# dsilvestro/npBNN

Hardware: AMD Instinct MI355X
Metric: MCMC iterations/sec (full fwd+lik per proposal) (higher is better)
Workload: dtype f16x3-split/f32

## Files before the change

npbnn_amd/csrc/npbnn_eval.hip.h:

```cpp
#pragma once
#include "npbnn_common.hip.h"
#include "npbnn_chain.hip.h"

namespace npbnn {

typedef void (*eval_fn_t)(const EvalParams*, int, int);
constexpr int kLikCat = 0, kLikGauss = 1, kLikGen = 2;
__host__ __device__ inline int lik_class(int lik_kind) {
    return lik_needs_row_scratch(lik_kind) ? kLikGen : (lik_kind == NPBNN_LIK_GAUSS ? kLikGauss : kLikCat);
}

template <int LK>
struct TileAcc {
    double ll;
};
template <>
struct TileAcc<kLikGauss> {
    double s1[4], s2[4];
};
constexpr int kFastGaussTargets = 2;

__device__ __forceinline__ int uni(int v) { return __builtin_amdgcn_readfirstlane(v); }
__device__ __forceinline__ float uni(float v) { return __uint_as_float(__builtin_amdgcn_readfirstlane(__float_as_uint(v))); }
__device__ __forceinline__ long long uni(long long v) {
    const unsigned lo = __builtin_amdgcn_readfirstlane((unsigned)(unsigned long long)v);
    const unsigned hi = __builtin_amdgcn_readfirstlane((unsigned)((unsigned long long)v >> 32));
    return (long long)(((unsigned long long)hi << 32) | lo);
}
template <typename T>
__device__ __forceinline__ T* uni(T* ptr) { return reinterpret_cast<T*>(uni((long long)reinterpret_cast<unsigned long long>(ptr))); }

#ifndef NPBNN_LAUNDER_TID
#define NPBNN_LAUNDER_TID (FAST && !SPEC && (BLK || (LK == kLikGauss && MT0 >= 2) || MT0 >= 3))
#endif
#ifndef NPBNN_LAUNDER_TAIL
#define NPBNN_LAUNDER_TAIL (FAST && !SPEC && (BLK || (LK == kLikGauss && MT0 >= 2) || MT0 >= 3))
#endif
#ifndef NPBNN_FAST3_WAVES
#define NPBNN_FAST3_WAVES 12
#endif
constexpr int kFastMaxMT0 = 4;
constexpr int kFastLayers = 3;
struct HotParams {
    const int* labels;
    const float* targets;
    const float* inst_w;
    unsigned* confusion;
    float* y_out;
    long long n_rows;
    int use_classw, predict_mode, weight_sets;
    int aux_off_w, aux_off_t;
    int n_layers, C, MTL, lik_kind, k_targets, act_kind, out_kind, final_act, classw_off, pad_masked;
    int slope_off;
    int l1_f16;
    int frag_off[kFastLayers - 1], bias_off[kFastLayers - 1], in_live[kFastLayers - 1];
    float act_prm[kFastLayers - 1];
};

template <int KIND, int HT, int D>
__device__ __forceinline__ void act_tiles_all(f32x4 (&h)[D][HT], int live, float prm) {
#pragma unroll
    for (int mt = 0; mt < HT; ++mt)
        if (mt < live)
#pragma unroll
            for (int i = 0; i < 4; ++i)
#pragma unroll
                for (int j = 0; j < D; ++j) h[j][mt][i] = act_apply(h[j][mt][i], KIND, prm);
}
template <int HT, int D>
__device__ __forceinline__ void act_live_all(f32x4 (&h)[D][HT], int live, int kind, float prm) {
    switch (kind) {
        case NPBNN_ACT_RELU: act_tiles_all<NPBNN_ACT_RELU>(h, live, prm); break;
        case NPBNN_ACT_LEAKY: act_tiles_all<NPBNN_ACT_LEAKY>(h, live, prm); break;
        case NPBNN_ACT_SWISH: act_tiles_all<NPBNN_ACT_SWISH>(h, live, prm); break;
        default: act_tiles_all<NPBNN_ACT_TANH>(h, live, prm); break;
    }
}

template <int MT0, int MTI, int LK, int D, int DA, int J0, int NLC = 0, int ACTC = -1, bool PLAIN = false, bool F16IMG = false, int GT = 0>
__device__ __forceinline__ void tile_tail(const NetMeta& net, const HotParams& hp, const float* imgs0, int image_floats,
                                          const f32x4 (&acc0_all)[DA][MT0], int lane, int n, int kq, const char* a_slot, float* row_scratch,
                                          long long row, bool row_ok, TileAcc<LK> (&A_all)[DA]) {
    static_assert(J0 + D <= DA, "candidate range");
    constexpr bool primary = J0 == 0;
    const float* const imgs = imgs0 + (size_t)J0 * image_floats;
    auto A = [&](int j) -> TileAcc<LK>& { return A_all[J0 + j]; };
    constexpr int HT = MT0 > MTI ? MT0 : MTI;
    static_assert(NLC == 0 || (MTI == 1 && NLC >= 2 && NLC <= kFastLayers), "shape-specialised tails: 2..kFastLayers layers, narrow later layers");
    static_assert(!PLAIN || (NLC > 0 && LK != kLikGen), "the plain form needs a fixed shape");
    const int n_layers = NLC ? NLC : hp.n_layers;
    const int C = hp.C;
    const int MTL = NLC ? 1 : hp.MTL;
    const int lik_kind = (PLAIN && LK == kLikCat) ? NPBNN_LIK_CATEGORICAL : hp.lik_kind;
    const int k_targets = hp.k_targets;
    const bool need_softmax = LK == kLikCat && (PLAIN || (lik_kind == NPBNN_LIK_CATEGORICAL) || (hp.predict_mode == 2 && hp.out_kind == NPBNN_OUT_SOFTMAX));
    f32x4 h[D][HT];
#pragma unroll
    for (int j = 0; j < D; ++j)
#pragma unroll
        for (int mt = 0; mt < HT; ++mt) h[j][mt] = mt < MT0 ? acc0_all[J0 + j][mt < MT0 ? mt : 0] : f32x4{0.f, 0.f, 0.f, 0.f};
    auto layer = [&](int lkt, int lmt, int frag_off, int bias_off, float prm, int hidden, int live_s) {
        if constexpr (ACTC >= 0) {
            act_tiles_all<ACTC>(h, lkt, prm);
        } else if (hp.slope_off >= 0) {
#pragma unroll
            for (int j = 0; j < D; ++j) act_live(h[j], lkt, hp.act_kind, imgs[(size_t)j * image_floats + hp.slope_off + hidden]);
        } else {
            act_live_all(h, lkt, hp.act_kind, prm);
        }
        const float* frag = imgs + frag_off + lane * 4;
        const float* bias = imgs + bias_off + 4 * kq;
        f32x4 acc[D][MTI];
#pragma unroll
        for (int mt = 0; mt < MTI; ++mt) {
#pragma unroll
            for (int j = 0; j < D; ++j) acc[j][mt] = f32x4{0.f, 0.f, 0.f, 0.f};
            if (mt < lmt) {
#pragma unroll
                for (int j = 0; j < D; ++j) acc[j][mt] = *reinterpret_cast<const f32x4*>(bias + (size_t)j * image_floats + 16 * mt);
#pragma unroll
                for (int ct = 0; ct < HT; ++ct) {
                    if (ct < lkt) {
                        f32x4 a[D];
#pragma unroll
                        for (int j = 0; j < D; ++j)
                            a[j] = *reinterpret_cast<const f32x4*>(frag + (size_t)j * image_floats + (size_t)(ct * lmt + mt) * 256);
#pragma unroll
                        for (int s = 0; s < 4; ++s)
                            if (s < live_s)
#pragma unroll
                                for (int j = 0; j < D; ++j)
                                    acc[j][mt] = __builtin_amdgcn_mfma_f32_16x16x4f32(a[j][s], h[j][ct][s], acc[j][mt], 0, 0, 0);
                    }
                }
            }
        }
#pragma unroll
        for (int j = 0; j < D; ++j)
#pragma unroll
            for (int mt = 0; mt < MTI; ++mt) h[j][mt] = acc[j][mt];
    };
    constexpr bool L1F = F16IMG && MT0 >= 2 && MTI == 1 && (ACTC < 0 || ACTC == NPBNN_ACT_TANH);
    auto layer1_f16 = [&](int frag_off, int bias_off) {
        act_tiles_all<NPBNN_ACT_TANH>(h, MT0, 0.f);
        f32x4 acc[D];
#pragma unroll
        for (int j = 0; j < D; ++j) acc[j] = *reinterpret_cast<const f32x4*>(imgs + (size_t)j * image_floats + bias_off + 4 * kq);
#pragma unroll
        for (int q = 0; q < (MT0 + 1) / 2; ++q) {
            f16x8 xh[D], xl[D];
#pragma unroll
            for (int j = 0; j < D; ++j)
#pragma unroll
                for (int e = 0; e < 8; ++e) {
                    const int t = 2 * q + (e >> 2);
                    const float x = t < MT0 ? h[j][t < MT0 ? t : 0][e & 3] : 0.f;
                    const _Float16 hi = (_Float16)x;
                    xh[j][e] = hi;
                    xl[j][e] = (_Float16)(x - (float)hi);
                }
#pragma unroll
            for (int j = 0; j < D; ++j) {
                const float* fr = imgs + (size_t)j * image_floats + frag_off + q * 512 + lane * 4;
                const f16x8 wh = *reinterpret_cast<const f16x8*>(fr);
                const f16x8 wl = *reinterpret_cast<const f16x8*>(fr + 256);
                acc[j] = __builtin_amdgcn_mfma_f32_16x16x32_f16(wh, xh[j], acc[j], 0, 0, 0);
                acc[j] = __builtin_amdgcn_mfma_f32_16x16x32_f16(wl, xh[j], acc[j], 0, 0, 0);
                acc[j] = __builtin_amdgcn_mfma_f32_16x16x32_f16(wh, xl[j], acc[j], 0, 0, 0);
            }
        }
#pragma unroll
        for (int j = 0; j < D; ++j) h[j][0] = acc[j];
    };
    if constexpr (NLC > 0) {
        if constexpr (L1F) {
            if (hp.l1_f16) layer1_f16(hp.frag_off[0], hp.bias_off[0]);
            else layer(MT0, 1, hp.frag_off[0], hp.bias_off[0], hp.act_prm[0], 0, hp.in_live[0]);
#pragma unroll
            for (int l = 2; l < NLC; ++l) layer(1, 1, hp.frag_off[l - 1], hp.bias_off[l - 1], hp.act_prm[l - 1], l - 1, hp.in_live[l - 1]);
        } else {
#pragma unroll
        for (int l = 1; l < NLC; ++l) layer(l == 1 ? MT0 : 1, 1, hp.frag_off[l - 1], hp.bias_off[l - 1], hp.act_prm[l - 1], l - 1, hp.in_live[l - 1]);
        }
    } else {
        for (int l = 1; l < n_layers; ++l) {
            const LayerMeta& L = net.L[l];
            if constexpr (L1F) {
                if (l == 1 && hp.l1_f16) { layer1_f16(uni(L.frag_off), uni(L.bias_off)); continue; }
            }
            layer(uni(L.kt), uni(L.mt), uni(L.frag_off), uni(L.bias_off), uni(net.act_prm[l - 1]), l - 1, uni(L.in_live));
        }
    }
    if (!PLAIN && hp.final_act) act_live_all(h, MTL, hp.act_kind, uni(net.act_prm[n_layers - 1]));

    float lse[D];
    int best_i = 0;
#pragma unroll
    for (int j = 0; j < D; ++j) lse[j] = 0.f;
    if (need_softmax) {
        float m[D], se[D];
#pragma unroll
        for (int j = 0; j < D; ++j) { m[j] = -INFINITY; se[j] = 0.f; }
        if (PLAIN || hp.pad_masked) {
#pragma unroll
            for (int mt = 0; mt < MTI; ++mt)
                if (mt < MTL)
#pragma unroll
                    for (int i = 0; i < 4; ++i)
#pragma unroll
                        for (int j = 0; j < D; ++j) m[j] = max_nn(m[j], h[j][mt][i]);
#pragma unroll
            for (int j = 0; j < D; ++j) m[j] = quad_max(m[j]);
#pragma unroll
            for (int mt = 0; mt < MTI; ++mt)
                if (mt < MTL)
#pragma unroll
                    for (int i = 0; i < 4; ++i)
#pragma unroll
                        for (int j = 0; j < D; ++j) {
                            const float e = __expf(h[j][mt][i] - m[j]);
                            se[j] = (mt == 0 && i == 0) ? e : se[j] + e;
                        }
        } else {
#pragma unroll
            for (int mt = 0; mt < MTI; ++mt)
                if (mt < MTL)
#pragma unroll
                    for (int i = 0; i < 4; ++i)
                        if (16 * mt + 4 * kq + i < C)
#pragma unroll
                            for (int j = 0; j < D; ++j) m[j] = max_nn(m[j], h[j][mt][i]);
#pragma unroll
            for (int j = 0; j < D; ++j) m[j] = quad_max(m[j]);
#pragma unroll
            for (int mt = 0; mt < MTI; ++mt)
                if (mt < MTL)
#pragma unroll
                    for (int i = 0; i < 4; ++i)
                        if (16 * mt + 4 * kq + i < C)
#pragma unroll
                            for (int j = 0; j < D; ++j) se[j] += __expf(h[j][mt][i] - m[j]);
        }
#pragma unroll
        for (int j = 0; j < D; ++j) se[j] = quad_sum(se[j]);
#pragma unroll
        for (int j = 0; j < D; ++j) lse[j] = m[j] + log_1_to_n(se[j]);
        if (!PLAIN && hp.confusion && primary) {
            float bv = -INFINITY;
            int bi = 0x7fffffff;
#pragma unroll
            for (int mt = 0; mt < MTI; ++mt)
                if (mt < MTL)
#pragma unroll
                    for (int i = 0; i < 4; ++i) {
                        const int o = 16 * mt + 4 * kq + i;
                        if (o < C && h[0][mt][i] > bv) { bv = h[0][mt][i]; bi = o; }
                    }
            quad_argmax(bv, bi);
            best_i = bi;
        }
    }

    if constexpr (LK == kLikCat) {
      if (lik_kind == NPBNN_LIK_CATEGORICAL) {
        const int lab = *reinterpret_cast<const int*>(a_slot + n * 4);
        float zl[D];
        bool own = false;
#pragma unroll
        for (int j = 0; j < D; ++j) zl[j] = 0.f;
#pragma unroll
        for (int mt = 0; mt < MTI; ++mt)
            if (mt < MTL)
#pragma unroll
                for (int i = 0; i < 4; ++i)
                    if (16 * mt + 4 * kq + i == lab) {
                        own = true;
#pragma unroll
                        for (int j = 0; j < D; ++j) zl[j] = h[j][mt][i];
                    }
        if (lab >= 0) {
            float wgt = 1.f;
            if constexpr (!PLAIN) {
                if (hp.inst_w) wgt *= *reinterpret_cast<const float*>(a_slot + hp.aux_off_w + n * 4);
                if (hp.use_classw) wgt *= imgs[hp.classw_off + lab];
            }
#pragma unroll
            for (int j = 0; j < D; ++j) {
                float term = 0.f;
                if (own) term += zl[j];
                if (kq == 0) term -= lse[j];
                if constexpr (!PLAIN) term *= wgt;
                A(j).ll += (double)term;
            }
            if (!PLAIN && hp.confusion && primary && kq == 0 && best_i < C) atomicAdd(hp.confusion + lab * C + best_i, 1u);
        }
      }
    } else if constexpr (LK == kLikGen) {
        const float* tg = reinterpret_cast<const float*>(a_slot + hp.aux_off_t);
#pragma unroll
        for (int c = 0; c < D; ++c) {
            *reinterpret_cast<f32x4*>(row_scratch + n * 16 + 4 * kq) = h[c][0];
            double term = 0.0;
            if (row_ok) {
                for (int j = kq; j < k_targets; j += 4) {
                    const double y = (double)tg[n * k_targets + j];
                    if (lik_kind == NPBNN_LIK_GAUSS_PRED_SIGMA) {
                        const double mu = (double)row_scratch[n * 16 + j];
                        const double zs = (double)row_scratch[n * 16 + k_targets + j];
                        const double sg = fmax(zs, 0.0) + log1p(exp(-fabs(zs)));
                        const double r = (y - mu) / sg;
                        term += -0.9189385332046727418 - log(sg) - 0.5 * r * r;
                    } else if (lik_kind == NPBNN_LIK_POISSON) {
                        if (j == 0) {
                            const double eta = (double)row_scratch[n * 16];
                            term += y * eta - exp(eta) - lgamma(y + 1.0);
                        }
                    } else {
                        const bool one_col = lik_kind != NPBNN_LIK_NEGBIN2D;
                        if (one_col && j > 0) continue;
                        const int jp = one_col ? 1 : k_targets + j;
                        const double e0 = (double)row_scratch[n * 16 + j], e1 = (double)row_scratch[n * 16 + jp];
                        double mean, pr;
                        if (lik_kind == NPBNN_LIK_NEGBIN_BASE10) {
                            mean = exp(2.302585092994046 * e0);
                            pr = 1.0 / (1.0 + exp(-2.302585092994046 * e1));
                        } else {
                            mean = exp(e0);
                            pr = 1.0 / (1.0 + exp(-e1));
                        }
                        const double nn = pr * mean / (1.0 - pr);
                        term += lgamma(y + nn) - lgamma(y + 1.0) - lgamma(nn) + nn * log(pr) + y * log1p(-pr);
                    }
                }
            }
            A(c).ll += term;
        }
    } else {
        const float* tg = reinterpret_cast<const float*>(a_slot + hp.aux_off_t);
        constexpr int GI = GT ? GT : (PLAIN ? kFastGaussTargets : 4);
#pragma unroll
        for (int i = 0; i < GI; ++i) {
            const int o = 4 * kq + i;
            if (o < k_targets && row_ok) {
                const float y = tg[n * k_targets + o];
#pragma unroll
                for (int j = 0; j < D; ++j) {
                    const float r = y - h[j][0][i];
                    A(j).s1[i] += (double)r;
                    A(j).s2[i] += (double)r * (double)r;
                }
            }
        }
    }

    if (!PLAIN && hp.predict_mode && row_ok) {
#pragma unroll
        for (int j = 0; j < D; ++j) {
            if (!(hp.weight_sets || (primary && j == 0))) continue;
            float* const yo = hp.y_out + (size_t)(J0 + j) * (size_t)hp.n_rows * C;
#pragma unroll
            for (int mt = 0; mt < MTI; ++mt)
                if (mt < MTL)
#pragma unroll
                    for (int i = 0; i < 4; ++i) {
                        const int o = 16 * mt + 4 * kq + i;
                        if (o < C) {
                            float v = h[j][mt][i];
                            if (hp.predict_mode == 2) {
                                if (hp.out_kind == NPBNN_OUT_SOFTMAX) v = __expf(v - lse[j]);
                                else if (hp.out_kind == NPBNN_OUT_SOFTPLUS_HALF && o >= C / 2) v = softplus_f(v);
                            }
                            yo[row * C + o] = v;
                        }
                    }
        }
    }
}

__host__ __device__ constexpr bool pipelined_l0(int mt0, int mti, bool f16, int d, bool fast_dense = false) {
    return f16 && mti == 1 && ((d == 3 && mt0 <= 2) || (d == 2 && (mt0 <= 1 || (fast_dense && (mt0 == 3 || mt0 == 4)))) || (d == 1 && mt0 <= 2));
}
__host__ __device__ constexpr int max_cand_for(int mt0) { return mt0 <= 2 ? 3 : 2; }
__host__ __device__ constexpr int max_waves_for(int mt0, int mti, bool f16, int d, int lk, bool fast = false) {
    return mti != 1 ? 8 : d == 1 ? 16 : d == 2 ? (fast ? 12 : 14) : fast ? (NPBNN_FAST3_WAVES) : (lk == kLikCat && pipelined_l0(mt0, mti, f16, d)) ? 13 : 11;
}
#define NPBNN_WAIT_LGKM0() __builtin_amdgcn_s_waitcnt(0xc07f)

typedef int i32x16_t __attribute__((ext_vector_type(16)));
__device__ __forceinline__ void warm_scalar_cache(const EvalParams* pp) {
    static_assert(sizeof(EvalParams) <= 16 * 64, "one s_load_dwordx16 per 64-byte line");
    i32x16_t a, b, c, d;
    asm volatile(
        "s_load_dwordx16 %0, %4, 0x0\n\ts_load_dwordx16 %1, %4, 0x40\n\ts_load_dwordx16 %2, %4, 0x80\n\ts_load_dwordx16 %3, %4, 0xc0\n\t"
        "s_load_dwordx16 %0, %4, 0x100\n\ts_load_dwordx16 %1, %4, 0x140\n\ts_load_dwordx16 %2, %4, 0x180\n\ts_load_dwordx16 %3, %4, 0x1c0\n\t"
        "s_load_dwordx16 %0, %4, 0x200\n\ts_load_dwordx16 %1, %4, 0x240\n\ts_load_dwordx16 %2, %4, 0x280\n\ts_load_dwordx16 %3, %4, 0x2c0\n\t"
        "s_load_dwordx16 %0, %4, 0x300\n\ts_load_dwordx16 %1, %4, 0x340\n\ts_load_dwordx16 %2, %4, 0x380\n\t"
        "s_waitcnt lgkmcnt(0)"
        : "=&s"(a), "=&s"(b), "=&s"(c), "=&s"(d) : "s"(pp) : "memory");
}

template <int MT0, int MTI, bool F16, int D, int LK, bool FAST = false, bool BLK = false, bool CHAIN = true, bool SPEC = false>
__global__ void __launch_bounds__(max_waves_for(MT0, MTI, F16, D, LK, FAST) * 64) eval_kernel(const EvalParams* __restrict__ pp, int launch_arg, int n_loop) {
    static_assert(CHAIN || D == 1, "plain builds evaluate one weight set");
    static_assert(!SPEC || (CHAIN && FAST && !BLK), "spec builds: fast chain builds of dense first layers");
    static_assert(!FAST || (MTI == 1 && LK != kLikGen), "fast builds: narrow later layers, categorical or Gaussian likelihood");
    static_assert(!BLK || (FAST && MT0 >= 2), "block-structure builds are fast builds of layers with several output tiles");
    constexpr bool SKIP = !FAST || BLK;
    const int launch0 = launch_arg & 0x3fffffff;
    const bool next_enqueued = (launch_arg >> 30) & 1;
    const int launch_end = launch0 + (n_loop > 1 ? n_loop : 1);
#ifndef NPBNN_EXP_NO_WARM
    warm_scalar_cache(pp);
#endif
    const EvalParams& p = *pp;
    const int bid = uni((int)blockIdx.x);
    unsigned long long* const stamps = uni(p.stamps);
#define NPBNN_ESTAMP(k) do { if (stamps && threadIdx.x == 0) stamps[(size_t)bid * 8 + (k)] = wall_clock64(); } while (0)
#ifdef NPBNN_EXP_PROLOGUE_STAMPS
#define NPBNN_ESTAMPX(k) do { if (stamps && threadIdx.x == 0) stamps[(size_t)gridDim.x * 24 + (size_t)bid * 8 + (k)] = wall_clock64(); } while (0)
#else
#define NPBNN_ESTAMPX(k) do { } while (0)
#endif
    constexpr int DEPTH = F16 ? ((kRing - 1) & ~1) : kRing - 1;
    constexpr bool PIPE = pipelined_l0(MT0, MTI, F16, D, FAST && !BLK && !SPEC) && kRing == 4;
    extern __shared__ __attribute__((aligned(16))) char smem[];
    const ChainParams* const chain = CHAIN ? uni(p.chain) : nullptr;
    const int GN = (CHAIN && D > 1) ? uni(p.group_n) : 0;
    const int G = (int)gridDim.x - (GN ? GN : chain ? 1 : 0);
    if (GN && bid >= G) {
        StepShared& sh = *reinterpret_cast<StepShared*>(smem);
        chain_step(*uni(p.group[bid - G].chain), overlapped_plan(launch0), sh);
        return;
    }
    const bool sync = chain && uni(p.sync_mode);
    const int ebid = sync ? bid - 1 : bid;
    const int share_rot = (CHAIN && sync && !GN) ? uni(p.share_rot) : 0;
    int lbid = ebid;
    for (int i = 0; i < launch0 && share_rot > 0; ++i) { lbid += share_rot; if (lbid >= G) lbid -= G; }
    if (chain && bid == (sync ? 0 : G)) {
        StepShared& sh = *reinterpret_cast<StepShared*>(smem);
        int* const lds_flag = reinterpret_cast<int*>(smem + sizeof(StepShared));
        if (SPEC && uni(p.sync_mode) == 3) {
            SpecShared& sp = *reinterpret_cast<SpecShared*>(smem + ((sizeof(StepShared) + 64 + 15) & ~(size_t)15));
            if (chain->mask) spec_rounds<true>(*chain, launch0, launch_end, G, sh, sp, lds_flag);
            else spec_rounds<false>(*chain, launch0, launch_end, G, sh, sp, lds_flag);
            return;
        }
        for (int launch = launch0; launch < launch_end; ++launch) {
            if (sync && !sync_step_enter(*chain, launch, G, lds_flag)) return;
            chain_step(*chain, overlapped_plan(launch), sh);
            if (sync) sync_step_leave(chain->st, launch + 1, next_enqueued && launch + 1 == launch_end);
            if (launch + 1 < launch_end) {
                __syncthreads();
                if (threadIdx.x == 0) {
                    const PassDesc& nx = chain->pass[overlapped_plan(launch).out];
                    *lds_flag = (nx.n_cand == 0 && nx.pad[0] == 1) ? 1 : 0;
                }
                __syncthreads();
                if (*lds_flag) return;
                __syncthreads();
            }
        }
        return;
    }
#ifdef NPBNN_EXP_PROLOGUE_STAMPS
    unsigned long long t_prev_pass0 = 0;
#endif
    constexpr bool LOOK = CHAIN && !SPEC;
    int ahead_t0 = -1;
    int ahead_cnt[D];
#pragma unroll
    for (int j = 0; j < D; ++j) ahead_cnt[j] = 0;
    for (int launch = launch0; launch < launch_end; ++launch, lbid = (lbid + share_rot >= G ? lbid + share_rot - G : lbid + share_rot)) {
#ifdef NPBNN_EXP_PROLOGUE_STAMPS
    const unsigned long long t_pass0 = stamps ? wall_clock64() : 0;
#else
    NPBNN_ESTAMP(0);
#endif
    const EvalParams* pp_pass = pp;
    asm volatile("" : "+s"(pp_pass));
    typedef const __attribute__((address_space(4))) EvalParams ConstEvalParams;
    ConstEvalParams& p = *(ConstEvalParams*)pp_pass;
    const EvalParams& p_generic = *pp_pass;
    typedef const __attribute__((address_space(4))) ChainParams ConstChainParams;
    ChainDev* const st_dev = chain ? uni(((ConstChainParams*)chain)->st) : nullptr;
    const SpecState* const spec_dev = (SPEC && chain) ? uni(((ConstChainParams*)chain)->spec) : nullptr;
    unsigned long long* const spec_part = (SPEC && chain) ? uni(((ConstChainParams*)chain)->spec_part) : nullptr;
    const unsigned spec_gen0 = (SPEC && chain) ? (unsigned)uni(((ConstChainParams*)chain)->spec_gen) : 0u;
    int tid_pass = threadIdx.x;
    if constexpr (NPBNN_LAUNDER_TID) asm volatile("" : "+v"(tid_pass));
    const int tid = tid_pass;
    const int lane = tid & 63;
    const int wave = __builtin_amdgcn_readfirstlane(tid >> 6);
    const int n = lane & 15, kq = lane >> 4;
    const auto& net = p.net;
    const NetMeta& net_generic = p_generic.net;
    const int wpb = blockDim.x >> 6;
    const int image_floats = uni(net.image_floats);
    const size_t IB = (size_t)image_floats * 4;

    HotParams hp;
    hp.n_layers = uni(net.n_layers); hp.C = uni(net.n_out);
    hp.k_targets = uni(net.k_targets); hp.act_kind = uni(net.act_kind);
#pragma unroll
    for (int l = 1; l < kFastLayers; ++l) { hp.frag_off[l - 1] = 0; hp.bias_off[l - 1] = 0; hp.act_prm[l - 1] = 0.f; hp.in_live[l - 1] = 4; }
    if constexpr (FAST) {
        hp.labels = LK == kLikCat ? uni(p.labels) : nullptr;
        hp.targets = LK == kLikGauss ? uni(p.targets) : nullptr;
        hp.inst_w = nullptr; hp.confusion = nullptr; hp.y_out = nullptr;
        hp.n_rows = LK == kLikGauss ? uni(p.n_rows) : 0;
        hp.use_classw = 0; hp.predict_mode = 0; hp.weight_sets = 0;
        hp.MTL = 1; hp.lik_kind = LK == kLikGauss ? NPBNN_LIK_GAUSS : NPBNN_LIK_CATEGORICAL;
        hp.out_kind = 0; hp.final_act = 0; hp.pad_masked = 1; hp.classw_off = -1; hp.slope_off = -1;
        hp.l1_f16 = uni(net.l1_f16);
#pragma unroll
        for (int l = 1; l < kFastLayers; ++l)
            if (l < hp.n_layers) {
                hp.frag_off[l - 1] = uni(net.L[l].frag_off);
                hp.bias_off[l - 1] = uni(net.L[l].bias_off);
                hp.act_prm[l - 1] = uni(net.act_prm[l - 1]);
                hp.in_live[l - 1] = uni(net.L[l].in_live);
            }
    } else {
        hp.labels = uni(p.labels); hp.targets = uni(p.targets); hp.inst_w = uni(p.inst_w); hp.confusion = uni(p.confusion);
        hp.y_out = uni(p.y_out);
        hp.n_rows = uni(p.n_rows); hp.use_classw = uni(p.use_classw); hp.predict_mode = uni(p.predict_mode);
        hp.weight_sets = uni(p.weight_sets);
        hp.MTL = uni(net.L[hp.n_layers - 1].mt); hp.lik_kind = uni(net.lik_kind);
        hp.out_kind = uni(net.out_kind);
        hp.final_act = uni(net.final_act);
        hp.pad_masked = uni(net.pad_masked);
        hp.classw_off = uni(net.classw_off);
        hp.slope_off = uni(p.cand_slopes) != nullptr ? uni(net.slope_off) : -1;
        hp.l1_f16 = uni(net.l1_f16);
    }
    const int k_targets = hp.k_targets;
    const int aux_sz = uni(p.lay.aux_sz), aux_mask = uni(p.lay.aux_slots) - 1;
    hp.aux_off_w = uni(p.lay.off_w);
    hp.aux_off_t = uni(p.lay.off_t);
    const float* const Xg = uni(p.X);
    const int Fp = uni(p.Fp);
    const int n_tiles = uni(p.n_tiles);
    const int M = uni(p.M);
    const int* const g_pos = uni(p.pos);
    const float* const g_pscale = uni(p.pscale);
    double* const g_partials = uni(p.partials);

    NPBNN_ESTAMPX(0);
    char* const ring = smem + D * IB + (size_t)wave * uni(p.lay.wave_lds);
    char* const aux = ring + kRing * 1024;
    float* const row_scratch = reinterpret_cast<float*>(aux + (aux_mask + 1) * aux_sz);

    auto stage_images = [&]() {
        const int n_pieces = (image_floats + 255) >> 8;
        const float* const image = uni(p.image);
        const size_t set_stride = hp.weight_sets ? (size_t)image_floats : 0;
        const float* img[D];
#pragma unroll
        for (int j = 0; j < D; ++j) img[j] = GN ? uni(p.group[j].image) : image + j * set_stride;
        auto copy_all = [&](auto coherent) {
            for (int i = wave; i < n_pieces; i += wpb)
                if (i * 256 + lane * 4 < image_floats) {
#pragma unroll
                    for (int j = 0; j < D; ++j) {
                        if constexpr (decltype(coherent)::value) dma16_coherent(img[j] + (size_t)i * 256 + lane * 4, smem + j * IB + (size_t)i * 1024);
                        else dma16(img[j] + (size_t)i * 256 + lane * 4, smem + j * IB + (size_t)i * 1024);
                    }
                }
        };
        if (sync) copy_all(std::true_type{});
        else copy_all(std::false_type{});
    };

    const int KT0 = uni(net.L[0].kt);
    const int first_tile = lbid + G * wave;
    const int simd_waves = (wpb - (wave & 3) + 3) >> 2;
    const int stride = G * 4 * simd_waves;
    int my_tiles = 0;
    if (first_tile < n_tiles) {
        if (n_tiles - first_tile <= 32 * stride) {
            for (int t = first_tile; t < n_tiles; t += stride) ++my_tiles;
        } else {
            my_tiles = (n_tiles - first_tile + stride - 1) / stride;
        }
    }
    const int Q = my_tiles * KT0;
    int Dp = PIPE ? kRing : DEPTH;
    if (Dp > 2 * KT0) Dp = 2 * KT0;
    const bool full_depth = (Dp == DEPTH);

    const float* pf_ptr = Xg + (size_t)first_tile * 16 * (size_t)Fp;
    const unsigned pf_lane = ((unsigned)n * (unsigned)Fp + 4u * (unsigned)kq) * 4u;
    const size_t tile_jump = (size_t)stride * 16 * (size_t)Fp - (size_t)KT0 * 16;
    int pf_q = 0, pf_kt = 0, pf_tile = first_tile, pf_seq = 0, pf_slot = 0;
    auto issue_aux = [&]() {
        char* a = aux + (pf_seq & aux_mask) * aux_sz;
        const size_t r0 = (size_t)pf_tile * 16;
        if (lane < 16) {
            if (hp.labels) dma4(hp.labels + r0 + lane, a);
            if (hp.inst_w) dma4(hp.inst_w + r0 + lane, a + hp.aux_off_w);
        }
        if (hp.targets) {
            const int total = 16 * k_targets;
            for (int e = 0; e < total; e += 64) {
                const int idx = e + lane;
                if (idx < total)
                    dma4(hp.targets + r0 * k_targets + idx, a + hp.aux_off_t + e * 4);
            }
        }
    };
    auto issue_next = [&]() {
        if (pf_kt == 0) issue_aux();
        dma16(reinterpret_cast<const float*>(reinterpret_cast<const char*>(pf_ptr) + pf_lane), ring + pf_slot);
        pf_ptr += 16;
        pf_slot = ring_next(pf_slot);
        ++pf_q;
        if (++pf_kt == KT0) { pf_kt = 0; pf_tile += stride; ++pf_seq; pf_ptr += tile_jump; }
    };
    auto issue_pair = [&]() {
        if (pf_kt == 0) issue_aux();
        const float* const g = reinterpret_cast<const float*>(reinterpret_cast<const char*>(pf_ptr) + pf_lane);
        dma16(g, ring + pf_slot);
        __builtin_amdgcn_global_load_lds((gvoid*)g, (lvoid*)(ring + pf_slot + (1024 - 64)), 16, 64, 0);
        pf_ptr += 32;
        pf_slot += 2048;
        if (pf_slot == kRing * 1024) pf_slot = 0;
        pf_q += 2;
        pf_kt += 2;
        if (pf_kt == KT0) { pf_kt = 0; pf_tile += stride; ++pf_seq; pf_ptr += tile_jump; }
    };
    auto issue_first = [&](int depth) {
        if constexpr (F16) {
            static_assert(kRing <= 4, "one statement per pair of ring slots");
            if (0 < depth && pf_q < Q) issue_pair();
            if (2 < depth && pf_q < Q) issue_pair();
        } else {
            for (int i = 0; i < depth && pf_q < Q; ++i) issue_next();
        }
    };
    const bool early_copy = SPEC && uni(p.sync_mode) == 3;
    if (early_copy) {
        stage_images();
        issue_first(Dp);
    }

    const bool ahead = LOOK && ahead_t0 >= 0;
    int early_prepared = 0x7fffffff;
    if (sync && !ahead && !early_copy && threadIdx.x == 0)
        early_prepared = __hip_atomic_load(&st_dev->prepared, __ATOMIC_RELAXED, __HIP_MEMORY_SCOPE_AGENT);
    const int par = (chain || GN) ? (launch & 1) : 0;
    int t0 = 0;
    int cnt[D];
    int t0g[D];
#pragma unroll
    for (int j = 0; j < D; ++j) { cnt[j] = 0; t0g[j] = 0; }
    const PassDesc* const pass = (CHAIN && uni(p.has_pass)) ? &p_generic.pass_desc[par] : nullptr;
    int pv_slot = par, acc_cnt = 0, acc_slot = -1;
    int* const wait_words = reinterpret_cast<int*>(smem + D * IB + (size_t)wpb * uni(p.lay.wave_lds));
    bool entered = true;
    if constexpr (SPEC) {
        if (early_copy) entered = sync_eval_enter_spec(st_dev, spec_dev, p_generic.pass_desc, launch, par, wait_words);
        else if (sync && !ahead) entered = sync_eval_enter(st_dev, launch, wait_words, early_prepared);
    } else {
        if (sync && !ahead) entered = sync_eval_enter(st_dev, launch, wait_words, early_prepared);
    }
    if (!entered) {
        if constexpr (SPEC) NPBNN_WAIT_VMCNT(0);
        return;
    }
    asm volatile("" :: "v"(early_prepared));
    if (GN) {
        int alive = 0;
#pragma unroll
        for (int j = 0; j < D; ++j) {
            const PassDesc* const dj = uni(p.group[j].pass) + par;
            const int nc = uni(dj->n_cand);
            alive |= nc;
            cnt[j] = nc > 0 ? uni(dj->cnt[0]) : 0;
            t0g[j] = uni(dj->t0);
        }
        if (!alive) return;
    } else if (pass && ahead) {
        t0 = ahead_t0;
#pragma unroll
        for (int j = 0; j < D; ++j) cnt[j] = ahead_cnt[j];
    } else if (pass) {
        if (sync) {
            const int w = (SPEC && early_copy) ? wait_words[lane & 7]
                                               : __hip_atomic_load(reinterpret_cast<const int*>(pass) + (lane & 7), __ATOMIC_RELAXED, __HIP_MEMORY_SCOPE_AGENT);
            if (__builtin_amdgcn_readlane(w, 1) == 0) {
                if (threadIdx.x == 0) sync_eval_leave(st_dev, launch);
                if (n_loop <= 1 || __builtin_amdgcn_readlane(w, 5) == 1 || (SPEC && uni(p.sync_mode) == 3)) {
                    if constexpr (SPEC) NPBNN_WAIT_VMCNT(0);
                    return;
                }
                if constexpr (SPEC) NPBNN_WAIT_VMCNT(0);
                __syncthreads();
                continue;
            }
            t0 = __builtin_amdgcn_readlane(w, 0);
#pragma unroll
            for (int j = 0; j < D; ++j) cnt[j] = __builtin_amdgcn_readlane(w, 2 + (j < kMaxCand ? j : 0));
            if (SPEC && uni(p.sync_mode) == 3) {
                acc_cnt = __builtin_amdgcn_readlane(w, 6);
                const int named = __builtin_amdgcn_readlane(w, 7);
                pv_slot = named & 0xff;
                acc_slot = (named >> 8) - 1;
            }
        } else {
            const auto& cpass = p.pass_desc[par];
            if (uni(cpass.n_cand) == 0) return;
            t0 = uni(cpass.t0);
#pragma unroll
            for (int j = 0; j < D; ++j) cnt[j] = uni(cpass.cnt[j < kMaxCand ? j : 0]);
        }
    }

    NPBNN_ESTAMPX(1);
    if (!early_copy) {
        if (!ahead) stage_images();
        NPBNN_ESTAMPX(2);
        issue_first(Dp);
    }
    ahead_t0 = -1;
    NPBNN_ESTAMPX(3);
    const double* const pv = uni(p.pv) + (size_t)pv_slot * kMaxCand * M;
    const int* const void_flag = chain ? uni(&st_dev->void_launch) : nullptr;
    int void_seen = -3;
    int ppos[D];
    double pval[D];
    float psc[D];
    auto patch_src = [&](int j, const int*& pos_row, const float*& psc_row, const double*& pv_row) {
        if (GN) {
            const int Mj = uni(p.group[j].M);
            const float* const sc = uni(p.group[j].pscale);
            pos_row = uni(p.group[j].pos) + (size_t)t0g[j] * Mj;
            psc_row = sc ? sc + (size_t)t0g[j] * Mj : nullptr;
            pv_row = uni(p.group[j].pv) + (size_t)par * kMaxCand * Mj;
        } else {
            pos_row = g_pos + (size_t)(t0 + j) * M;
            psc_row = g_pscale ? g_pscale + (size_t)(t0 + j) * M : nullptr;
            pv_row = pv + (size_t)j * M;
        }
    };
    {
        typedef const __attribute__((address_space(1))) int gint_t;
        typedef const __attribute__((address_space(1))) float gfloat_t;
        typedef const __attribute__((address_space(1))) double gdouble_t;
        const int* pos_rows[D]; const float* psc_rows[D]; const double* pv_rows[D];
#pragma unroll
        for (int j = 0; j < D; ++j) {
            pos_rows[j] = nullptr; psc_rows[j] = nullptr; pv_rows[j] = nullptr;
            if (pass || GN) patch_src(j, pos_rows[j], psc_rows[j], pv_rows[j]);
        }
#pragma unroll
        for (int j = 0; j < D; ++j) {
            ppos[j] = 0; pval[j] = 0.0; psc[j] = 1.0f;
            if ((pass || GN) && tid < cnt[j]) {
                ppos[j] = ((gint_t*)pos_rows[j])[tid];
                pval[j] = sync ? __hip_atomic_load((gdouble_t*)pv_rows[j] + tid, __ATOMIC_RELAXED, __HIP_MEMORY_SCOPE_AGENT) : ((gdouble_t*)pv_rows[j])[tid];
                if (psc_rows[j]) psc[j] = ((gfloat_t*)psc_rows[j])[tid];
            }
        }
    }
    int apos = kSkipPos;
    double aval = 0.0;
    float asc = 1.0f;
    if constexpr (!SPEC) acc_cnt = 0;
    if (acc_cnt > 0 && tid < acc_cnt) {
        const size_t arow = (size_t)(t0 - 1) * M;
        apos = g_pos[arow + tid];
        aval = __hip_atomic_load(uni(p.pv) + (size_t)acc_slot * M + tid, __ATOMIC_RELAXED, __HIP_MEMORY_SCOPE_AGENT);
        if (g_pscale) asc = g_pscale[arow + tid];
    }
#ifdef NPBNN_EXP_PROLOGUE_STAMPS
    if (stamps && threadIdx.x == 0) {
        stamps[(size_t)bid * 8] = t_pass0;
        stamps[(size_t)gridDim.x * 24 + (size_t)bid * 8 + 5] = t_prev_pass0;
    }
    t_prev_pass0 = t_pass0;
#endif
    NPBNN_ESTAMP(1);
    __syncthreads();
    NPBNN_ESTAMP(2);
#pragma unroll
    for (int j = 0; j < D; ++j) asm volatile("" : "+v"(ppos[j]), "+v"(pval[j]), "+v"(psc[j]));
    const int l0_rows_img = MT0 >= 3 ? uni(net.l0_rows) : 16;
    auto lo_halves = [&](int pos) { return (MT0 >= 3 && (pos & kPosCompact)) ? 32 * l0_rows_img : 512; };
    if (acc_cnt > 0) {
        auto put = [&](int pos, double v, float sc) {
            if (pos == kSkipPos) return;
#pragma unroll
            for (int j = 0; j < D; ++j) {
                float* imgj = reinterpret_cast<float*>(smem + j * IB);
                if (pos < 0) {
                    _Float16 hi, lo;
                    split_f16((float)(v * (double)sc), hi, lo);
                    _Float16* i16 = reinterpret_cast<_Float16*>(imgj);
                    const int hpos = pos & 0x3fffffff;
                    i16[hpos] = hi;
                    i16[hpos + lo_halves(pos)] = lo;
                } else {
                    imgj[pos] = (float)v;
                }
            }
        };
        if (tid < acc_cnt) put(apos, aval, asc);
        if ((int)blockDim.x < acc_cnt) {
            const size_t arow = (size_t)(t0 - 1) * M;
            for (int e = tid + blockDim.x; e < acc_cnt; e += blockDim.x)
                put(g_pos[arow + e], __hip_atomic_load(uni(p.pv) + (size_t)acc_slot * M + e, __ATOMIC_RELAXED, __HIP_MEMORY_SCOPE_AGENT),
                    g_pscale ? g_pscale[arow + e] : 1.0f);
        }
        __syncthreads();
    }
    if (pass || GN) {
        auto patch = [&](int j, int pos, double v, float sc) {
            if (pos == 0x7fffffff) return;
            float* imgj = reinterpret_cast<float*>(smem + j * IB);
            if (pos < 0) {
                _Float16 hi, lo;
                split_f16((float)(v * (double)sc), hi, lo);
                _Float16* i16 = reinterpret_cast<_Float16*>(imgj);
                const int hpos = pos & 0x3fffffff;
                i16[hpos] = hi;
                i16[hpos + lo_halves(pos)] = lo;
            } else {
                imgj[pos] = (float)v;
            }
        };
        if (hp.slope_off >= 0 && tid < D * kMaxLayers) {
            const int j = tid / kMaxLayers, l = tid % kMaxLayers;
            const double* src = uni(p.cand_slopes) + ((size_t)par * kMaxCand + j) * kMaxLayers + l;
            reinterpret_cast<float*>(smem + j * IB)[hp.slope_off + l] =
                (float)(sync ? __hip_atomic_load(src, __ATOMIC_RELAXED, __HIP_MEMORY_SCOPE_AGENT) : *src);
        }
#pragma unroll
        for (int j = 0; j < D; ++j) {
            if (tid < cnt[j]) patch(j, ppos[j], pval[j], psc[j]);
            if ((int)blockDim.x < cnt[j]) {
                const int* pos_row; const float* psc_row; const double* pv_row;
                patch_src(j, pos_row, psc_row, pv_row);
                for (int e = tid + blockDim.x; e < cnt[j]; e += blockDim.x)
                    patch(j, pos_row[e], sync ? __hip_atomic_load(pv_row + e, __ATOMIC_RELAXED, __HIP_MEMORY_SCOPE_AGENT) : pv_row[e],
                          psc_row ? psc_row[e] : 1.0f);
            }
        }
        __syncthreads();
    }
    NPBNN_ESTAMP(3);

    TileAcc<LK> A[D];
    constexpr int GI = FAST ? (BLK ? 1 : kFastGaussTargets) : 4;
#pragma unroll
    for (int j = 0; j < D; ++j) {
        if constexpr (LK == kLikGauss) {
#pragma unroll
            for (int i = 0; i < GI; ++i) { A[j].s1[i] = 0.0; A[j].s2[i] = 0.0; }
        } else {
            A[j].ll = 0.0;
        }
    }

    const float* const imgs = reinterpret_cast<const float*>(smem);
    const int l0_rows = (F16 && MT0 >= 3) ? uni(net.l0_rows) : 16;
    const int slot_f = (F16 && MT0 >= 3) ? 32 * l0_rows : 512, lo_f = (F16 && MT0 >= 3) ? 16 * l0_rows : 256;
    const int frag0_off = uni(net.L[0].frag_off) + ((F16 && MT0 >= 3) ? (kq * l0_rows + (n < l0_rows ? n : l0_rows - 1)) * 4 : lane * 4);
    const int bias0_off = uni(net.L[0].bias_off) + 4 * kq;
    int ub[MT0], ue[MT0], uo[MT0];
#pragma unroll
    for (int mt = 0; mt < MT0; ++mt) {
        ub[mt] = uni(net.l0_begin[mt]);
        ue[mt] = uni(net.l0_end[mt]);
        uo[mt] = uni(net.l0_base[mt]) - ub[mt];
    }
    auto unit_tiles = [&](int u) {
        if constexpr (!SKIP) return (1 << MT0) - 1;
        int m = 0;
#pragma unroll
        for (int mt = 0; mt < MT0; ++mt) m |= (u >= ub[mt] && u < ue[mt]) ? (1 << mt) : 0;
        return m;
    };
    auto load_bias0 = [&](f32x4 (&acc0)[D][MT0]) {
#pragma unroll
        for (int j = 0; j < D; ++j)
#pragma unroll
            for (int mt = 0; mt < MT0; ++mt)
                acc0[j][mt] = *reinterpret_cast<const f32x4*>(imgs + (size_t)j * image_floats + bias0_off + 16 * mt);
    };
    auto run_tail = [&](const f32x4 (&acc0)[D][MT0], int tseq, int tile) {
#ifdef NPBNN_EXP_NO_TAIL
        if constexpr (LK != kLikGauss) {
#pragma unroll
            for (int j = 0; j < D; ++j) A[j].ll += (double)acc0[j][0][0];
        }
        return;
#endif
        const char* a_slot = aux + (tseq & aux_mask) * aux_sz;
        int lane_t = lane;
        if constexpr (NPBNN_LAUNDER_TAIL) asm volatile("" : "+v"(lane_t));
        const int n = lane_t & 15, kq = lane_t >> 4;
        const int lane = lane_t;
        const long long row = (long long)tile * 16 + n;
        constexpr int HT = MT0 > MTI ? MT0 : MTI;
        constexpr int DT = (D * HT <= 6 && LK != kLikGen) ? D : 1;
        auto tail = [&](auto nlc, auto actc, auto plain) {
            constexpr int NLC = decltype(nlc)::value, ACTC = decltype(actc)::value;
            constexpr bool PL = decltype(plain)::value;
            if constexpr (DT == D) {
                tile_tail<MT0, MTI, LK, D, D, 0, NLC, ACTC, PL, F16, GI>(net_generic, hp, imgs, image_floats, acc0, lane, n, kq, a_slot, row_scratch, row, row < hp.n_rows, A);
            } else {
                tile_tail<MT0, MTI, LK, 1, D, 0, NLC, ACTC, PL, F16, GI>(net_generic, hp, imgs, image_floats, acc0, lane, n, kq, a_slot, row_scratch, row, row < hp.n_rows, A);
                if constexpr (D > 1) tile_tail<MT0, MTI, LK, 1, D, 1, NLC, ACTC, PL, F16, GI>(net_generic, hp, imgs, image_floats, acc0, lane, n, kq, a_slot, row_scratch, row, row < hp.n_rows, A);
                if constexpr (D > 2) tile_tail<MT0, MTI, LK, 1, D, 2, NLC, ACTC, PL, F16, GI>(net_generic, hp, imgs, image_floats, acc0, lane, n, kq, a_slot, row_scratch, row, row < hp.n_rows, A);
                static_assert(D <= 3, "add a call per candidate");
            }
        };
        using std::integral_constant;
        if constexpr (FAST) {
            auto with_act = [&](auto nlc) {
                switch (hp.act_kind) {
                    case NPBNN_ACT_RELU: tail(nlc, integral_constant<int, NPBNN_ACT_RELU>{}, std::true_type{}); break;
                    case NPBNN_ACT_LEAKY: tail(nlc, integral_constant<int, NPBNN_ACT_LEAKY>{}, std::true_type{}); break;
                    case NPBNN_ACT_SWISH: tail(nlc, integral_constant<int, NPBNN_ACT_SWISH>{}, std::true_type{}); break;
                    default: tail(nlc, integral_constant<int, NPBNN_ACT_TANH>{}, std::true_type{}); break;
                }
            };
            static_assert(kFastLayers == 3, "one branch per specialised depth");
            if (hp.n_layers == 3) with_act(integral_constant<int, 3>{});
            else with_act(integral_constant<int, 2>{});
        } else {
            tail(integral_constant<int, 0>{}, integral_constant<int, -1>{}, std::false_type{});
        }
    };

    if constexpr (PIPE) {
        struct WFrag { f16x8 wh[MT0], wl[MT0]; };
        struct XFrag { f16x8 xh, xl; };
        const int KS = KT0 >> 1;
        const int S = my_tiles * KS;
        if (S > 0) {
            WFrag Wb[2];
            XFrag Xb[2];
            f32x4 acc0[D][MT0];
            int ld_slot = 0;
            int s = 0, ks = 0;
            static_assert(kRing == 4, "a K-step is two ring slots: the steps alternate between slots (0, 1) and (2, 3)");
            const unsigned x_lane = (unsigned)(D * IB) + (unsigned)wave * (unsigned)uni(p.lay.wave_lds)
                                    + (unsigned)((kq >> 1) * 1024 + ((2 * (kq & 1)) * 16 + n) * 16);
            unsigned w_lane[D];
#pragma unroll
            for (int j = 0; j < D; ++j) w_lane[j] = (unsigned)(j * IB) + (unsigned)frag0_off * 4u;
            auto load_x = [&](XFrag& x) {
                const char* px = smem + (x_lane + (unsigned)ld_slot);
                x.xh = *reinterpret_cast<const f16x8*>(px);
                x.xl = *reinterpret_cast<const f16x8*>(px + 256);
                ld_slot ^= 2048;
            };
            auto load_w = [&](WFrag& w, int kstep, int j) {
                const unsigned slot_b = (unsigned)slot_f * 4u, lo_b = (unsigned)lo_f * 4u;
                const unsigned fr = w_lane[j] + (unsigned)kstep * slot_b;
                const int live = unit_tiles(kstep);
#pragma unroll
                for (int mt = 0; mt < MT0; ++mt)
                    if (live & (1 << mt)) {
                        const char* pw = smem + (fr + (unsigned)uo[mt] * slot_b);
                        w.wh[mt] = *reinterpret_cast<const f16x8*>(pw);
                        w.wl[mt] = *reinterpret_cast<const f16x8*>(pw + lo_b);
                    }
            };
            NPBNN_WAIT_VMCNT(0);
            load_x(Xb[0]);
            load_w(Wb[0], 0, 0);
            load_bias0(acc0);
            auto step = [&](auto par_tag) {
                constexpr int PAR = decltype(par_tag)::value;
                const int ks_next = (ks + 1 == KS) ? 0 : ks + 1;
                const int live = unit_tiles(ks);
                bool issued = false;
#pragma unroll
                for (int j = 0; j < D; ++j) {
                    const WFrag& wc = Wb[(PAR * D + j) & 1];
                    WFrag& wn = Wb[(PAR * D + j + 1) & 1];
                    NPBNN_WAIT_LGKM0();
                    if (j == 0 && pf_q < Q) {
                        issue_pair();
                        issued = true;
                    }
                    if (j == D - 1) {
                        if (s + 1 < S) {
                            if (issued) wait_depth<2>();
                            else NPBNN_WAIT_VMCNT(0);
                            load_x(Xb[PAR ^ 1]);
                            load_w(wn, ks_next, 0);
                        }
                    } else {
                        load_w(wn, ks, j + 1);
                    }
                    __builtin_amdgcn_sched_barrier(0);
#ifndef NPBNN_EXP_NO_L0
#pragma unroll
                    for (int mt = 0; mt < MT0; ++mt)
                        if (live & (1 << mt)) acc0[j][mt] = __builtin_amdgcn_mfma_f32_16x16x32_f16(wc.wh[mt], Xb[PAR].xh, acc0[j][mt], 0, 0, 0);
#pragma unroll
                    for (int mt = 0; mt < MT0; ++mt)
                        if (live & (1 << mt)) acc0[j][mt] = __builtin_amdgcn_mfma_f32_16x16x32_f16(wc.wl[mt], Xb[PAR].xh, acc0[j][mt], 0, 0, 0);
#pragma unroll
                    for (int mt = 0; mt < MT0; ++mt)
                        if (live & (1 << mt)) acc0[j][mt] = __builtin_amdgcn_mfma_f32_16x16x32_f16(wc.wh[mt], Xb[PAR].xl, acc0[j][mt], 0, 0, 0);
#else
                    acc0[j][0][0] += (float)wc.wh[0][0] + (float)wc.wl[MT0 - 1][7] + (float)Xb[PAR].xh[0] + (float)Xb[PAR].xl[7];
#endif
                    __builtin_amdgcn_sched_barrier(0);
                }
                ++s;
                ks = ks_next;
            };
            int tile = first_tile;
            unsigned long long tail_ticks = 0;
            for (int tseq = 0; tseq < my_tiles; ++tseq, tile += stride) {
                if (void_flag && void_seen == launch) break;
                for (int kp = 0; kp + 1 < KS; kp += 2) {
                    step(std::integral_constant<int, 0>{});
                    step(std::integral_constant<int, 1>{});
                }
                if (KS & 1) {
                    step(std::integral_constant<int, 0>{});
                    Xb[0] = Xb[1];
                    if (D & 1) Wb[0] = Wb[1];
                }
                const unsigned long long tk = stamps ? wall_clock64() : 0;
                if (void_flag) void_seen = __hip_atomic_load(void_flag, __ATOMIC_RELAXED, __HIP_MEMORY_SCOPE_AGENT);
                run_tail(acc0, tseq, tile);
                load_bias0(acc0);
                if (stamps) tail_ticks += wall_clock64() - tk;
            }
            if (stamps && tid == 0) stamps[(size_t)bid * 8 + 7] = tail_ticks;
        }
    } else {
    int q = 0, cs_slot = 0;
    int tile = first_tile;
    for (int tseq = 0; tseq < my_tiles; ++tseq, tile += stride) {
        if (void_flag && void_seen == launch) break;
        f32x4 acc0[D][MT0];
        load_bias0(acc0);
        int fr_off = frag0_off;
        int unit = 0;
        auto consume = [&]() {
            const int live = unit_tiles(unit);
            if constexpr (F16) {
                const int slot_b = ring_next(cs_slot);
                const char* px = ring + ((kq >> 1) ? slot_b : cs_slot) + ((2 * (kq & 1)) * 16 + n) * 16;
                const f16x8 xh = *reinterpret_cast<const f16x8*>(px);
                const f16x8 xl = *reinterpret_cast<const f16x8*>(px + 256);
                cs_slot = ring_next(slot_b);
#pragma unroll
                for (int j = 0; j < D; ++j) {
                    const float* fr = imgs + (size_t)j * image_floats + fr_off;
                    f16x8 wh[MT0], wl[MT0];
#pragma unroll
                    for (int mt = 0; mt < MT0; ++mt)
                        if (live & (1 << mt)) {
                            wh[mt] = *reinterpret_cast<const f16x8*>(fr + uo[mt] * slot_f);
                            wl[mt] = *reinterpret_cast<const f16x8*>(fr + uo[mt] * slot_f + lo_f);
                        }
#pragma unroll
                    for (int mt = 0; mt < MT0; ++mt)
                        if (live & (1 << mt)) acc0[j][mt] = __builtin_amdgcn_mfma_f32_16x16x32_f16(wh[mt], xh, acc0[j][mt], 0, 0, 0);
#pragma unroll
                    for (int mt = 0; mt < MT0; ++mt)
                        if (live & (1 << mt)) acc0[j][mt] = __builtin_amdgcn_mfma_f32_16x16x32_f16(wl[mt], xh, acc0[j][mt], 0, 0, 0);
#pragma unroll
                    for (int mt = 0; mt < MT0; ++mt)
                        if (live & (1 << mt)) acc0[j][mt] = __builtin_amdgcn_mfma_f32_16x16x32_f16(wh[mt], xl, acc0[j][mt], 0, 0, 0);
                }
                fr_off += slot_f;
                ++unit;
            } else {
                const f32x4 x = *reinterpret_cast<const f32x4*>(ring + cs_slot + lane * 16);
                cs_slot = ring_next(cs_slot);
#pragma unroll
                for (int j = 0; j < D; ++j) {
                    const float* fr = imgs + (size_t)j * image_floats + fr_off;
                    f32x4 a[MT0];
#pragma unroll
                    for (int mt = 0; mt < MT0; ++mt)
                        if (live & (1 << mt)) a[mt] = *reinterpret_cast<const f32x4*>(fr + uo[mt] * 256);
#pragma unroll
                    for (int s = 0; s < 4; ++s)
#pragma unroll
                        for (int mt = 0; mt < MT0; ++mt)
                            if (live & (1 << mt)) acc0[j][mt] = __builtin_amdgcn_mfma_f32_16x16x4f32(a[mt][s], x[s], acc0[j][mt], 0, 0, 0);
                }
                fr_off += 256;
                ++unit;
            }
        };
        constexpr int STEP = F16 ? 2 : 1;
        if (full_depth) {
            int n_issue = Q - pf_q;
            if (n_issue > KT0) n_issue = KT0;
            for (int kt = 0; kt < n_issue; kt += STEP) {
                if constexpr (F16) issue_pair();
                else issue_next();
                wait_depth<DEPTH>();
                consume();
            }
            if (n_issue < KT0) {
                NPBNN_WAIT_VMCNT(0);
                for (int kt = n_issue; kt < KT0; kt += STEP) consume();
            }
            q += KT0;
        } else {
            for (int kt = 0; kt < KT0; kt += STEP, q += STEP) {
                if (pf_q < Q) {
                    if constexpr (F16) issue_pair();
                    else issue_next();
                }
                wait_younger(pf_q - q - STEP);
                consume();
            }
        }

        if (void_flag) void_seen = __hip_atomic_load(void_flag, __ATOMIC_RELAXED, __HIP_MEMORY_SCOPE_AGENT);
        run_tail(acc0, tseq, tile);
    }
    }
    __builtin_amdgcn_s_waitcnt(0x0f70);
    const int tid_tiles = tid;
    {
    int tid_epi = tid_tiles;
    if constexpr (NPBNN_LAUNDER_TID) {
        tid_epi = threadIdx.x;
        asm volatile("" : "+v"(tid_epi));
    }
    const int tid = tid_epi;
    const int lane = tid & 63;
    const int n = lane & 15, kq = lane >> 4;

    NPBNN_ESTAMP(4);
    if (stamps && lane == 0) stamps[(size_t)gridDim.x * 8 + (size_t)bid * 16 + wave] = wall_clock64();
    const bool look = LOOK && sync && n_loop > 1 && launch + 1 < launch_end && !GN && g_partials != nullptr;
    int* const look_words = reinterpret_cast<int*>(smem + D * IB + (size_t)wpb * uni(p.lay.wave_lds));
    if (g_partials || GN) {
#pragma unroll
        for (int j = 0; j < D; ++j) {
            if constexpr (LK == kLikGauss) {
#pragma unroll
                for (int i = 0; i < GI; ++i) {
                    A[j].s1[i] = row_sum_f64(A[j].s1[i]);
                    A[j].s2[i] = row_sum_f64(A[j].s2[i]);
                }
            } else {
                A[j].ll = wave_sum_f64(A[j].ll);
            }
        }
        int nx_prepared = -1;
        if (look && wave == 0)
            nx_prepared = __hip_atomic_load(&st_dev->prepared, __ATOMIC_RELAXED, __HIP_MEMORY_SCOPE_AGENT);
        __syncthreads();
        NPBNN_ESTAMP(5);
        int nx_desc = 0;
        bool nx_ready = false;
        if (look && wave == 0) {
            nx_ready = uni(nx_prepared) >= launch + 1;
            if (nx_ready)
                nx_desc = __hip_atomic_load(reinterpret_cast<const int*>(&p_generic.pass_desc[(launch + 1) & 1]) + (lane & 7), __ATOMIC_RELAXED,
                                            __HIP_MEMORY_SCOPE_AGENT);
        }
        double* wsum = reinterpret_cast<double*>(smem + D * IB);
#pragma unroll
        for (int j = 0; j < D; ++j) {
            double* ws = wsum + ((size_t)j * wpb + wave) * kPartialStride;
            if constexpr (LK == kLikGauss) {
                if (lane == 0) ws[0] = 0.0;
                if (n == 0) {
#pragma unroll
                    for (int i = 0; i < 4; ++i) {
                        ws[1 + 4 * kq + i] = i < GI ? A[j].s1[i < GI ? i : 0] : 0.0;
                        ws[1 + NPBNN_MAX_TARGETS + 4 * kq + i] = i < GI ? A[j].s2[i < GI ? i : 0] : 0.0;
                    }
                }
            } else {
                if (lane == 0) ws[0] = A[j].ll;
            }
        }
        if (look && wave == 0 && lane < 8)
            look_words[lane] = nx_ready ? nx_desc : 0;
        asm volatile("" :: "v"(nx_prepared), "v"(nx_desc));
        __syncthreads();
        constexpr int nvals = (LK == kLikGauss) ? kPartialStride : 1;
        for (int item = tid - ((int)blockDim.x - 64); item >= 0 && item < D * nvals; item += 64) {
            const int j = item / nvals, v = item % nvals;
            if constexpr (LK == kLikGauss) { if (v != 0 && ((v - 1) & (NPBNN_MAX_TARGETS - 1)) >= p_generic.net.k_targets) continue; }
            double s = 0.0;
            for (int w = 0; w < wpb; ++w) s += wsum[((size_t)j * wpb + w) * kPartialStride + v];
            double* const dst = GN ? p.group[j].partials + (((size_t)par * kMaxCand) * kPartialStride + v) * G + lbid
                                   : g_partials + (((size_t)par * kMaxCand + j) * kPartialStride + v) * G + lbid;
            if constexpr (SPEC) {
                if (early_copy) { spec_part_store(spec_part + spec_part_index(par, j, v, lbid), s, spec_gen0 + (unsigned)launch + 1u); continue; }
            }
            if (sync) __hip_atomic_store(dst, s, __ATOMIC_RELAXED, __HIP_MEMORY_SCOPE_AGENT);
            else *dst = s;
        }
    }
    NPBNN_ESTAMP(6);
    if (sync) {
        __syncthreads();
        if (threadIdx.x == blockDim.x - 64 && !(SPEC && early_copy)) sync_eval_leave(st_dev, launch);
        if constexpr (LOOK) {
            if (look && look_words[1] > 0) {
                ahead_t0 = uni(look_words[0]);
#pragma unroll
                for (int j = 0; j < D; ++j) ahead_cnt[j] = uni(look_words[2 + (j < kMaxCand ? j : 0)]);
                stage_images();
            }
        }
    }
    }
    NPBNN_ESTAMPX(4);
    }
#undef NPBNN_ESTAMP
}

}
```

Measured before the change: 98870.

## Prefetch next launch's first X tiles during the partial-sum reduction epilogue

In look-ahead fast mode, each wave starts issuing the async global-to-LDS loads for the first ring slots of the next launch's input tiles during the current launch's reduction epilogue. The next iteration then only advances the prefetch counters (a dry run) instead of reissuing those loads. The wave-sum scratch is moved to the start of LDS so it does not overlap the ring. The goal is to hide the initial load latency at each launch boundary, at the cost of extra vmcnt drains on early-exit paths and tighter coupling between LDS layout and scheduling.

```diff
diff --git a/npbnn_amd/csrc/npbnn_eval.hip.h b/npbnn_amd/csrc/npbnn_eval.hip.h
--- a/npbnn_amd/csrc/npbnn_eval.hip.h
+++ b/npbnn_amd/csrc/npbnn_eval.hip.h
@@ -471,6 +471,8 @@
     int ahead_cnt[D];
 #pragma unroll
     for (int j = 0; j < D; ++j) ahead_cnt[j] = 0;
+    constexpr bool XA = LOOK && FAST;
+    bool x_ahead = false;
     for (int launch = launch0; launch < launch_end; ++launch, lbid = (lbid + share_rot >= G ? lbid + share_rot - G : lbid + share_rot)) {
 #ifdef NPBNN_EXP_PROLOGUE_STAMPS
     const unsigned long long t_pass0 = stamps ? wall_clock64() : 0;
@@ -584,7 +586,7 @@
             my_tiles = (n_tiles - first_tile + stride - 1) / stride;
         }
     }
-    const int Q = my_tiles * KT0;
+    int Q = my_tiles * KT0;
     int Dp = PIPE ? kRing : DEPTH;
     if (Dp > 2 * KT0) Dp = 2 * KT0;
     const bool full_depth = (Dp == DEPTH);
@@ -609,19 +611,24 @@
             }
         }
     };
-    auto issue_next = [&]() {
-        if (pf_kt == 0) issue_aux();
-        dma16(reinterpret_cast<const float*>(reinterpret_cast<const char*>(pf_ptr) + pf_lane), ring + pf_slot);
+    auto issue_next_as = [&](auto dry) {
+        if constexpr (!decltype(dry)::value) {
+            if (pf_kt == 0) issue_aux();
+            dma16(reinterpret_cast<const float*>(reinterpret_cast<const char*>(pf_ptr) + pf_lane), ring + pf_slot);
+        }
         pf_ptr += 16;
         pf_slot = ring_next(pf_slot);
         ++pf_q;
         if (++pf_kt == KT0) { pf_kt = 0; pf_tile += stride; ++pf_seq; pf_ptr += tile_jump; }
     };
-    auto issue_pair = [&]() {
-        if (pf_kt == 0) issue_aux();
-        const float* const g = reinterpret_cast<const float*>(reinterpret_cast<const char*>(pf_ptr) + pf_lane);
-        dma16(g, ring + pf_slot);
-        __builtin_amdgcn_global_load_lds((gvoid*)g, (lvoid*)(ring + pf_slot + (1024 - 64)), 16, 64, 0);
+    auto issue_next = [&]() { issue_next_as(std::false_type{}); };
+    auto issue_pair_as = [&](auto dry) {
+        if constexpr (!decltype(dry)::value) {
+            if (pf_kt == 0) issue_aux();
+            const float* const g = reinterpret_cast<const float*>(reinterpret_cast<const char*>(pf_ptr) + pf_lane);
+            dma16(g, ring + pf_slot);
+            __builtin_amdgcn_global_load_lds((gvoid*)g, (lvoid*)(ring + pf_slot + (1024 - 64)), 16, 64, 0);
+        }
         pf_ptr += 32;
         pf_slot += 2048;
         if (pf_slot == kRing * 1024) pf_slot = 0;
@@ -629,19 +636,20 @@
         pf_kt += 2;
         if (pf_kt == KT0) { pf_kt = 0; pf_tile += stride; ++pf_seq; pf_ptr += tile_jump; }
     };
-    auto issue_first = [&](int depth) {
+    auto issue_pair = [&]() { issue_pair_as(std::false_type{}); };
+    auto issue_first = [&](int depth, auto dry) {
         if constexpr (F16) {
             static_assert(kRing <= 4, "one statement per pair of ring slots");
-            if (0 < depth && pf_q < Q) issue_pair();
-            if (2 < depth && pf_q < Q) issue_pair();
+            if (0 < depth && pf_q < Q) issue_pair_as(dry);
+            if (2 < depth && pf_q < Q) issue_pair_as(dry);
         } else {
-            for (int i = 0; i < depth && pf_q < Q; ++i) issue_next();
+            for (int i = 0; i < depth && pf_q < Q; ++i) issue_next_as(dry);
         }
     };
     const bool early_copy = SPEC && uni(p.sync_mode) == 3;
     if (early_copy) {
         stage_images();
-        issue_first(Dp);
+        issue_first(Dp, std::false_type{});
     }
 
     const bool ahead = LOOK && ahead_t0 >= 0;
@@ -665,7 +673,7 @@
         if (sync && !ahead) entered = sync_eval_enter(st_dev, launch, wait_words, early_prepared);
     }
     if (!entered) {
-        if constexpr (SPEC) NPBNN_WAIT_VMCNT(0);
+        if constexpr (SPEC || XA) NPBNN_WAIT_VMCNT(0);
         return;
     }
     asm volatile("" :: "v"(early_prepared));
@@ -691,10 +699,11 @@
             if (__builtin_amdgcn_readlane(w, 1) == 0) {
                 if (threadIdx.x == 0) sync_eval_leave(st_dev, launch);
                 if (n_loop <= 1 || __builtin_amdgcn_readlane(w, 5) == 1 || (SPEC && uni(p.sync_mode) == 3)) {
-                    if constexpr (SPEC) NPBNN_WAIT_VMCNT(0);
+                    if constexpr (SPEC || XA) NPBNN_WAIT_VMCNT(0);
                     return;
                 }
-                if constexpr (SPEC) NPBNN_WAIT_VMCNT(0);
+                if constexpr (SPEC || XA) NPBNN_WAIT_VMCNT(0);
+                x_ahead = false;
                 __syncthreads();
                 continue;
             }
@@ -720,9 +729,11 @@
     if (!early_copy) {
         if (!ahead) stage_images();
         NPBNN_ESTAMPX(2);
-        issue_first(Dp);
+        if (XA && x_ahead) issue_first(Dp, std::true_type{});
+        else issue_first(Dp, std::false_type{});
     }
     ahead_t0 = -1;
+    x_ahead = false;
     NPBNN_ESTAMPX(3);
     const double* const pv = uni(p.pv) + (size_t)pv_slot * kMaxCand * M;
     const int* const void_flag = chain ? uni(&st_dev->void_launch) : nullptr;
@@ -1141,6 +1152,34 @@
     NPBNN_ESTAMP(4);
     if (stamps && lane == 0) stamps[(size_t)gridDim.x * 8 + (size_t)bid * 16 + wave] = wall_clock64();
     const bool look = LOOK && sync && n_loop > 1 && launch + 1 < launch_end && !GN && g_partials != nullptr;
+    const bool x_early = XA && look && (size_t)image_floats >= (size_t)wpb * kPartialStride * 2;
+    auto request_x_ahead = [&]() {
+        const EvalParams* pp_x = pp;
+        asm volatile("" : "+s"(pp_x));
+        ConstEvalParams& px = *(ConstEvalParams*)pp_x;
+        const int n_tiles_x = uni(px.n_tiles), kt0_x = uni(px.net.L[0].kt), fp_x = uni(px.Fp);
+        int nb = lbid + share_rot;
+        if (nb >= G) nb -= G;
+        const int ft = nb + G * wave;
+        int cnt = 0;
+        if (ft < n_tiles_x) {
+            if (n_tiles_x - ft <= 32 * stride) {
+                for (int t = ft; t < n_tiles_x; t += stride) ++cnt;
+            } else {
+                cnt = (n_tiles_x - ft + stride - 1) / stride;
+            }
+        }
+        Q = cnt * kt0_x;
+        pf_ptr = uni(px.X) + (size_t)ft * 16 * (size_t)fp_x;
+        pf_q = 0; pf_kt = 0; pf_tile = ft; pf_seq = 0; pf_slot = 0;
+        int depth = PIPE ? kRing : DEPTH;
+        if (depth > 2 * kt0_x) depth = 2 * kt0_x;
+        issue_first(depth, std::false_type{});
+    };
+    if constexpr (XA) {
+        if (x_early && wave != wpb - 1) request_x_ahead();
+        x_ahead = x_early;
+    }
     int* const look_words = reinterpret_cast<int*>(smem + D * IB + (size_t)wpb * uni(p.lay.wave_lds));
     if (g_partials || GN) {
 #pragma unroll
@@ -1168,7 +1207,7 @@
                 nx_desc = __hip_atomic_load(reinterpret_cast<const int*>(&p_generic.pass_desc[(launch + 1) & 1]) + (lane & 7), __ATOMIC_RELAXED,
                                             __HIP_MEMORY_SCOPE_AGENT);
         }
-        double* wsum = reinterpret_cast<double*>(smem + D * IB);
+        double* wsum = reinterpret_cast<double*>(x_early ? smem : smem + D * IB);
 #pragma unroll
         for (int j = 0; j < D; ++j) {
             double* ws = wsum + ((size_t)j * wpb + wave) * kPartialStride;
@@ -1209,6 +1248,7 @@
         __syncthreads();
         if (threadIdx.x == blockDim.x - 64 && !(SPEC && early_copy)) sync_eval_leave(st_dev, launch);
         if constexpr (LOOK) {
+            if constexpr (XA) { if (x_early && wave == wpb - 1) request_x_ahead(); }
             if (look && look_words[1] > 0) {
                 ahead_t0 = uni(look_words[0]);
 #pragma unroll
```

Result: slower. 97520 (-1.4%).
